# rohitgandikota/sliders

Measured on AMD Instinct MI355X. Metric: UNet denoise steps/sec (SDXL rank-4 text slider), higher is better.
Workload: dtype bf16; 1 GPU; sdxl text slider rank=4 alpha=1 noxattn+c3lier, 1024x1024, batch 1 (CFG pair), DDIM-50 partial denoise k~U{1..49} + 4 predictions + backward + AdamW; bench_step=one training iteration, prompt_pairs=8, parallelism=dp1

## Files before the change

### sliders_amd/csrc/lora.hip

```cpp
#include "addressing.h"
#include "../../include/sliders_hip.h"

namespace {

struct AddrArgs {
    const __bf16* a0; const __bf16* a1;
    int lda0, lda1, ca0, ca1;
    int mode, hs, ws, src_xform, stride, ho, wo;
};

template <int RMAX, int LPR>
__global__ __launch_bounds__(256) void skinny_kernel(AddrArgs A, const __bf16* __restrict__ w,
                                                     const __bf16* __restrict__ bias, void* out,
                                                     int M, int R, int K, int ldo, int out_kind, int kmajor) {
    const int tid = threadIdx.x;
    const int sub = tid & (LPR - 1);
    const int m = blockIdx.x * (256 / LPR) + tid / LPR;
    const bool active = m < M;
    const int mm = active ? m : M - 1;
    float acc[RMAX];
#pragma unroll
    for (int r = 0; r < RMAX; ++r) acc[r] = 0.f;
    const int cin = A.ca0 + A.ca1;

    auto fma_chunk = [&](const bf16x8 x, int k) {
        float xf[8];
#pragma unroll
        for (int e = 0; e < 8; ++e) xf[e] = (float)x[e];
        if (kmajor) {
            if (RMAX == 4) {
#pragma unroll
                for (int h = 0; h < 4; ++h) {
                    const bf16x8 wv = *(const bf16x8*)(w + (long)k * 4 + h * 8);
#pragma unroll
                    for (int r = 0; r < 4; ++r) {
                        acc[r] += xf[2 * h] * (float)wv[r];
                        acc[r] += xf[2 * h + 1] * (float)wv[4 + r];
                    }
                }
            }
            return;
        }
        bf16x8 wv[RMAX];
#pragma unroll
        for (int r = 0; r < RMAX; ++r) wv[r] = *(const bf16x8*)(w + (long)(r < R ? r : 0) * K + k);
#pragma unroll
        for (int r = 0; r < RMAX; ++r) {
            if (r < R) {
#pragma unroll
                for (int e = 0; e < 8; ++e) acc[r] += xf[e] * (float)wv[r][e];
            }
        }
    };

    if (A.mode == 0) {
        auto src_of = [&](int k) {
            const int kc = k < K ? k : 0;
            return kc < A.ca0 ? A.a0 + (long)mm * A.lda0 + kc : A.a1 + (long)mm * A.lda1 + (kc - A.ca0);
        };
        bf16x8 cur = *(const bf16x8*)src_of(sub * 8);
        for (int k = sub * 8; k < K; k += LPR * 8) {
            const bf16x8 nxt = *(const bf16x8*)src_of(k + LPR * 8);
            fma_chunk(cur, k);
            cur = nxt;
        }
    } else {
        const int hw = A.ho * A.wo;
        const int b = mm / hw;
        const int rem = mm - b * hw;
        const int oy = rem / A.wo, ox = rem - oy * A.wo;
        const int sh = A.src_xform ? 1 : 0;
        const int HL = A.hs << sh, WL = A.ws << sh;
        for (int tap = 0; tap < 9; ++tap) {
            const int ky = tap / 3, kx = tap - ky * 3;
            const int iy = oy * A.stride + ky - 1, ix = ox * A.stride + kx - 1;
            bool ok = (iy >= 0) & (iy < HL) & (ix >= 0) & (ix < WL);
            if (A.src_xform == 2) ok = ok & (((iy | ix) & 1) == 0);
            if (!ok) continue;
            const long pix = ((long)b * A.hs + (iy >> sh)) * A.ws + (ix >> sh);
            auto src_of = [&](int c) {
                const int cc = c < cin ? c : 0;
                return cc < A.ca0 ? A.a0 + pix * A.lda0 + cc : A.a1 + pix * A.lda1 + (cc - A.ca0);
            };
            bf16x8 cur = *(const bf16x8*)src_of(sub * 8);
            for (int c = sub * 8; c < cin; c += LPR * 8) {
                const bf16x8 nxt = *(const bf16x8*)src_of(c + LPR * 8);
                fma_chunk(cur, tap * cin + c);
                cur = nxt;
            }
        }
    }
#pragma unroll
    for (int r = 0; r < RMAX; ++r) {
#pragma unroll
        for (int o = LPR / 2; o > 0; o >>= 1) acc[r] += __shfl_xor(acc[r], o, 64);
    }
    if (active && sub == 0) {
        if (out_kind == 0) {
            float* o = (float*)out + (long)m * ldo;
#pragma unroll
            for (int r = 0; r < RMAX; ++r)
                if (r < R) o[r] = acc[r] + (bias ? (float)bias[r] : 0.f);
        } else {
            const int hw = A.ho * A.wo;
            const int b = m / hw;
            const int rem = m - b * hw;
            __bf16* o = (__bf16*)out;
#pragma unroll
            for (int r = 0; r < RMAX; ++r)
                if (r < R) o[((long)b * R + r) * hw + rem] = (__bf16)(acc[r] + (bias ? (float)bias[r] : 0.f));
        }
    }
}

__global__ __launch_bounds__(256) void gemv_kernel(const slh_gemv_desc d) {
    const int lane = threadIdx.x & 63;
    const int n = blockIdx.x * 4 + (threadIdx.x >> 6);
    if (n >= d.N) return;
    const __bf16* x = (const __bf16*)d.x;
    const __bf16* w = (const __bf16*)d.w + (long)n * d.K;
    float acc[8];
#pragma unroll
    for (int b = 0; b < 8; ++b) acc[b] = 0.f;
    for (int k = lane * 8; k < d.K; k += 512) {
        const bf16x8 wv = *(const bf16x8*)(w + k);
        bf16x8 xv[8];
#pragma unroll
        for (int b = 0; b < 8; ++b) xv[b] = *(const bf16x8*)(x + (long)(b < d.nb ? b : d.nb - 1) * d.ldx + k);
        float wf[8];
#pragma unroll
        for (int e = 0; e < 8; ++e) wf[e] = (float)wv[e];
#pragma unroll
        for (int b = 0; b < 8; ++b) {
            if (b < d.nb) {
#pragma unroll
                for (int e = 0; e < 8; ++e) {
                    float xe = (float)xv[b][e];
                    if (d.in_act == 1) xe = round_bf16(silu_f(xe));
                    acc[b] += xe * wf[e];
                }
            }
        }
    }
#pragma unroll
    for (int b = 0; b < 8; ++b) acc[b] = wave_sum(acc[b]);
    if (lane == 0) {
        const float bias = d.bias ? (float)((const __bf16*)d.bias)[n] : 0.f;
        float up[4] = {0.f, 0.f, 0.f, 0.f};
        float ls = 0.f;
        int tcol = 0;
        if (d.lora_t) {
            ls = *d.lora_scale;
            tcol = d.lora_tcol ? d.lora_tcol[n] : 0;
            const bf16x4 u = *(const bf16x4*)((const __bf16*)d.lora_up + (long)n * 4);
#pragma unroll
            for (int r = 0; r < 4; ++r) up[r] = (float)u[r];
        }
        for (int b = 0; b < d.nb; ++b) {
            float v = acc[b] + bias;
            if (d.lora_t) {
                const float* t = d.lora_t + (long)b * d.ld_t + tcol;
                v += ls * (t[0] * up[0] + t[1] * up[1] + t[2] * up[2] + t[3] * up[3]);
            }
            if (d.addend) v = round_bf16(v) + (float)((const __bf16*)d.addend)[(long)b * d.ld_add + n];
            if (d.out_f32) ((float*)d.y)[(long)b * d.ldy + n] = v;
            else ((__bf16*)d.y)[(long)b * d.ldy + n] = (__bf16)v;
        }
    }
}

struct WgradArgs {
    AddrArgs A;
    const float* v; float* out; const float* scale;
    int M, R, ldv, ldo, rows_per_block, rmajor, vgroup_cols;
    float* ws; unsigned* ticket;
};

template <int R>
__device__ __forceinline__ void wgrad_body(const WgradArgs& p, const int bx, const int by, const int bz, const long slab_id = 0,
                                           const int slab_step = 0, const long ticket_id = 0, const int splits = 1) {
    __shared__ float red[4][32][8 * R + 1];
    __shared__ int last_flag;
    const int cx = threadIdx.x & 31, ry = threadIdx.x >> 5;
    const int C = p.A.ca0 + p.A.ca1;
    const int c = (bx * 32 + cx) * 8;
    const bool cvalid = c < C;
    const int tap = bz;
    const int m_begin = by * p.rows_per_block;
    const int m_end = min(p.M, m_begin + p.rows_per_block);
    float acc[8][R];
#pragma unroll
    for (int e = 0; e < 8; ++e)
#pragma unroll
        for (int r = 0; r < R; ++r) acc[e][r] = 0.f;
    const int voff = p.vgroup_cols > 0 ? 4 * (c / p.vgroup_cols) : 0;
    const int ky = tap / 3, kx = tap - ky * 3;
    const SrcSel zs = src_select(p.A, c);
    if (cvalid) {
        for (int m = m_begin + ry; m < m_end; m += 8) {
            long pix = m;
            if (p.A.mode != 0) {
                const RowPixel px = pixel_of_row(m, p.A.ho, p.A.wo);
                const ConvTap t = conv_tap(p.A, px.b, px.oy, px.ox, ky, kx);
                if (!t.ok) continue;
                pix = t.pix;
            }
            const bf16x8 z = *(const bf16x8*)(zs.base + pix * zs.ld + zs.cc);
            float vv[R];
#pragma unroll
            for (int r = 0; r < R; ++r) vv[r] = p.v[(long)m * p.ldv + voff + r];
#pragma unroll
            for (int e = 0; e < 8; ++e) {
                const float ze = (float)z[e];
#pragma unroll
                for (int r = 0; r < R; ++r) acc[e][r] += ze * vv[r];
            }
        }
    }
#pragma unroll
    for (int e = 0; e < 8; ++e)
#pragma unroll
        for (int r = 0; r < R; ++r) {
            acc[e][r] += __shfl_xor(acc[e][r], 32, 64);
            if ((threadIdx.x & 32) == 0) red[threadIdx.x >> 6][cx][e * R + r] = acc[e][r];
        }
    __syncthreads();
    const float s = *p.scale;
    if (p.ws != nullptr) {
        constexpr int PER = 32 * 8 * R;
        const __amdgpu_buffer_rsrc_t slabs = __builtin_amdgcn_make_buffer_rsrc(p.ws + slab_id * PER - (long)by * slab_step * PER, 0,
                                                                              (int)((long)splits * slab_step * PER * 4), 0x00020000);
#pragma unroll
        for (int q = 0; q < PER / 1024; ++q) {
            const int idx = (q * 256 + threadIdx.x) * 4;
            f32x4 t4;
#pragma unroll
            for (int u = 0; u < 4; ++u) {
                const int ccx = (idx + u) / (8 * R), er = (idx + u) - ccx * (8 * R);
                float t = 0.f;
#pragma unroll
                for (int y = 0; y < 4; ++y) t += red[y][ccx][er];
                t4[u] = t;
            }
            __builtin_amdgcn_raw_buffer_store_b128(__builtin_bit_cast(u32x4, t4), slabs, (by * slab_step * PER + idx) * 4, 0, 16 );
        }
        if (!last_arriver(p.ticket + ticket_id, (unsigned)splits, &last_flag)) return;
#pragma unroll
        for (int q = 0; q < PER / 1024; ++q) {
            const int idx = (q * 256 + threadIdx.x) * 4;
            f32x4 tot = {0.f, 0.f, 0.f, 0.f};
            for (int k0 = 0; k0 < splits; k0 += 8) {
                f32x4 v[8];
#pragma unroll
                for (int u = 0; u < 8; ++u)
                    v[u] = k0 + u < splits ? __builtin_bit_cast(f32x4, __builtin_amdgcn_raw_buffer_load_b128(
                                                 slabs, ((k0 + u) * slab_step * PER + idx) * 4, 0, 16 ))
                                           : f32x4{0.f, 0.f, 0.f, 0.f};
#pragma unroll
                for (int u = 0; u < 8; ++u) tot += v[u];
            }
#pragma unroll
            for (int u = 0; u < 4; ++u) {
                const int ccx = (idx + u) / (8 * R), er = (idx + u) - ccx * (8 * R);
                const int e = er / R, r = er - e * R;
                const int cc = (bx * 32 + ccx) * 8 + e;
                if (cc >= C) continue;
                const long col = (p.A.mode == 0 ? 0 : (long)tap * C) + cc;
                float* o = p.rmajor ? p.out + (long)r * p.ldo + col : p.out + col * p.ldo + r;
                *o += s * tot[u];
            }
        }
        return;
    }
    for (int idx = threadIdx.x; idx < 32 * 8 * R; idx += 256) {
        const int ccx = idx / (8 * R);
        const int er = idx - ccx * (8 * R);
        const int e = er / R, r = er - e * R;
        const int cc = (bx * 32 + ccx) * 8 + e;
        if (cc >= C) continue;
        float t = 0.f;
#pragma unroll
        for (int y = 0; y < 4; ++y) t += red[y][ccx][er];
        const long col = (p.A.mode == 0 ? 0 : (long)tap * C) + cc;
        float* o = p.rmajor ? p.out + (long)r * p.ldo + col : p.out + col * p.ldo + r;
        atomicAdd(o, s * t);
    }
}

template <int R>
__global__ __launch_bounds__(256) void wgrad_kernel(const WgradArgs p) {
    wgrad_body<R>(p, blockIdx.x, blockIdx.y, blockIdx.z, ((long)blockIdx.z * gridDim.y + blockIdx.y) * gridDim.x + blockIdx.x,
                  (int)gridDim.x, (long)blockIdx.z * gridDim.x + blockIdx.x, (int)gridDim.y);
}

struct WgradGeom { int gx, splits, taps, rows_per_block; };
__host__ __device__ inline WgradGeom wgrad_geom(int C, int M, int mode, int kind) {
    WgradGeom g;
    g.gx = (C / 8 + 31) / 32;
    g.taps = mode == 1 ? 9 : 1;
    const int blocks_xz = g.gx * g.taps;
    const int target = kind == 0 ? 768 : 256;
    int splits = kind == 2 ? (M + 511) / 512 : (target + blocks_xz - 1) / blocks_xz;
    const int max_splits = (M + 63) / 64, min_splits = kind == 2 ? 1 : (M + 1023) / 1024;
    if (splits > max_splits) splits = max_splits;
    if (splits < min_splits) splits = min_splits;
    if (splits < 1) splits = 1;
    g.splits = splits;
    g.rows_per_block = ((M + splits - 1) / splits + 7) / 8 * 8;
    return g;
}

__host__ __device__ inline void fill_addr(AddrArgs& A, const void* a0, const void* a1, int lda0, int lda1, int ca0, int ca1, int mode,
                                         int hs, int ws, int src_xform, int stride, int ho, int wo) {
    A.a0 = (const __bf16*)a0; A.a1 = (const __bf16*)a1;
    A.lda0 = lda0; A.lda1 = lda1; A.ca0 = ca0; A.ca1 = ca1; A.mode = mode;
    A.hs = hs; A.ws = ws; A.src_xform = src_xform; A.stride = stride; A.ho = ho; A.wo = wo;
}

__host__ __device__ inline void wgrad_args(WgradArgs& p, const slh_wgrad_desc& d) {
    fill_addr(p.A, d.z0, d.z1, d.ldz0, d.ldz1, d.c0, d.c1, d.mode, d.hs, d.ws, d.src_xform, d.stride, d.ho, d.wo);
    p.v = d.v; p.out = d.out; p.scale = d.scale;
    p.M = d.M; p.R = d.R; p.ldv = d.ldv; p.ldo = d.ldo;
    p.rmajor = d.out_rmajor;
    p.vgroup_cols = d.vgroup_cols;
    p.ws = d.slabs; p.ticket = (unsigned*)d.tickets;
    p.rows_per_block = wgrad_geom(d.c0 + d.c1, d.M, d.mode, d.slabs ? 1 : 0).rows_per_block;
}

template <int R>
__global__ __launch_bounds__(256) void wgrad_batch_kernel(const slh_wgrad_desc* table, const int* prefix, int n, float* ws, unsigned* ticket) {
    const int bid = blockIdx.x;
    const int pi = __builtin_amdgcn_readfirstlane(batch_find(prefix, n, bid));
    const slh_wgrad_desc d = table[pi];
    WgradArgs p;
    wgrad_args(p, d);
    p.ws = ws; p.ticket = ticket;
    const WgradGeom g = wgrad_geom(d.c0 + d.c1, d.M, d.mode, ws ? 2 : 0);
    p.rows_per_block = g.rows_per_block;
    const int local = bid - prefix[pi];
    const int bx = local % g.gx, rest = local / g.gx;
    const int by = rest % g.splits, bz = rest / g.splits;
    wgrad_body<R>(p, bx, by, bz, bid, g.gx, (long)prefix[pi] + (long)bz * g.splits * g.gx + bx, g.splits);
}

}

struct skinny_form { int rmax, lpr, grid; };
static skinny_form skinny_choose(int M, int R) {
    skinny_form f;
    f.rmax = R <= 4 ? 4 : R <= 12 ? 12 : 16;
    f.lpr = M <= 16384 ? 64 : 16;
    const int rows = 256 / f.lpr;
    f.grid = (M + rows - 1) / rows;
    return f;
}

extern "C" int slh_skinny(const slh_skinny_desc* d, slh_stream_t stream) {
    SLH_CHECK(d && d->a0 && d->w && d->out, "slh_skinny: null pointer");
    SLH_CHECK(d->M > 0 && d->R > 0 && d->R <= 16 && d->K > 0, "slh_skinny: bad shape");
    SLH_CHECK(d->ca0 % 8 == 0 && d->ca1 % 8 == 0 && d->lda0 % 8 == 0 && d->lda1 % 8 == 0 && d->K % 8 == 0,
              "slh_skinny: 16-byte alignment");
    SLH_CHECK((d->a1 != nullptr) == (d->ca1 > 0), "slh_skinny: a1/ca1 mismatch");
    const int cin = d->ca0 + d->ca1;
    if (d->mode == 0) SLH_CHECK(cin == d->K, "slh_skinny: dense K mismatch");
    else {
        SLH_CHECK(d->mode == 1 && d->K == 9 * cin, "slh_skinny: conv K mismatch");
        SLH_CHECK(d->M == d->batch * d->ho * d->wo, "slh_skinny: conv M mismatch");
        SLH_CHECK(d->stride == 1 || d->stride == 2, "slh_skinny: stride");
    }
    if (d->out_kind == 1) SLH_CHECK(d->mode == 1, "slh_skinny: NCHW output needs conv geometry");
    if (d->w_kmajor) SLH_CHECK(d->R == 4 && d->mode == 0 && !d->bias, "slh_skinny: w_kmajor needs dense R=4");
    AddrArgs A;
    fill_addr(A, d->a0, d->a1, d->lda0, d->lda1, d->ca0, d->ca1, d->mode, d->hs, d->ws, d->src_xform, d->stride,
              d->ho, d->wo);
    hipStream_t s = (hipStream_t)stream;
    const skinny_form f = skinny_choose(d->M, d->R);
#define SLH_SKINNY_LAUNCH(RM, LPR)                                                                                 \
    do {                                                                                                           \
        if (slh_name_mode()) slh_name_record("skinny<%d,%d>", RM, LPR);                                            \
        else                                                                                                       \
            hipLaunchKernelGGL((skinny_kernel<RM, LPR>), dim3(f.grid), dim3(256), 0, s, A, (const __bf16*)d->w,    \
                               (const __bf16*)d->bias, d->out, d->M, d->R, d->K, d->ldo, d->out_kind, d->w_kmajor); \
    } while (0)
#define SLH_SKINNY_ROWS(RM)                                                                                        \
    do {                                                                                                           \
        if (f.lpr == 64) SLH_SKINNY_LAUNCH(RM, 64);                                                                \
        else SLH_SKINNY_LAUNCH(RM, 16);                                                                            \
    } while (0)
    if (f.rmax == 4) SLH_SKINNY_ROWS(4);
    else if (f.rmax == 12) SLH_SKINNY_ROWS(12);
    else SLH_SKINNY_ROWS(16);
#undef SLH_SKINNY_ROWS
#undef SLH_SKINNY_LAUNCH
    SLH_LAUNCH_CHECK("slh_skinny");
    return 0;
}

extern "C" int slh_skinny_kernel_name(const slh_skinny_desc* d, char* buf, int cap) {
    SLH_CHECK(buf && cap >= 32, "slh_skinny_kernel_name: buffer");
    slh_name_sink_set(buf, cap);
    const int rc = slh_skinny(d, nullptr);
    slh_name_sink_set(nullptr, 0);
    if (rc == 0 && !buf[0]) { slh_set_error("slh_skinny_kernel_name: internal: no launch site recorded a name"); return -3; }
    return rc;
}

extern "C" int slh_gemv(const slh_gemv_desc* d, slh_stream_t stream) {
    SLH_CHECK(d && d->x && d->w && d->y, "slh_gemv: null pointer");
    SLH_CHECK(d->nb >= 1 && d->nb <= 8 && d->N > 0 && d->K > 0 && d->K % 8 == 0 && d->ldx % 8 == 0,
              "slh_gemv: bad shape nb=%d N=%d K=%d", d->nb, d->N, d->K);
    if (d->lora_t) SLH_CHECK(d->lora_up && d->lora_scale, "slh_gemv: lora pointers");
    hipLaunchKernelGGL(gemv_kernel, dim3((d->N + 3) / 4), dim3(256), 0, (hipStream_t)stream, *d);
    SLH_LAUNCH_CHECK("slh_gemv");
    return 0;
}

static int wgrad_check(const slh_wgrad_desc* d, bool ptrs = true) {
    SLH_CHECK(d, "slh_lora_wgrad: null descriptor");
    if (ptrs) SLH_CHECK(d->z0 && d->v && d->out && d->scale, "slh_lora_wgrad: null pointer");
    SLH_CHECK(d->R == 4 || d->R == 12, "slh_lora_wgrad: R must be 4 or 12");
    SLH_CHECK(d->c0 % 8 == 0 && d->c1 % 8 == 0 && d->ldz0 % 8 == 0 && d->ldz1 % 8 == 0, "slh_lora_wgrad: alignment");
    if (ptrs) SLH_CHECK((d->z1 != nullptr) == (d->c1 > 0), "slh_lora_wgrad: z1/c1 mismatch");
    SLH_CHECK(d->M > 0 && d->c0 + d->c1 > 0, "slh_lora_wgrad: empty problem");
    if (d->mode == 1) SLH_CHECK(d->M == d->batch * d->ho * d->wo, "slh_lora_wgrad: conv M mismatch");
    if (d->vgroup_cols > 0)
        SLH_CHECK(d->vgroup_cols % 8 == 0 && (d->c0 + d->c1) % d->vgroup_cols == 0 && d->R == 4,
                  "slh_lora_wgrad: vgroup_cols %d needs a multiple of 8 that divides C = %d, and R = 4 (R = %d)", d->vgroup_cols,
                  d->c0 + d->c1, d->R);
    SLH_CHECK(d->vgroup_cols >= 0, "slh_lora_wgrad: negative vgroup_cols");
    return 0;
}

extern "C" int slh_lora_wgrad(const slh_wgrad_desc* d, slh_stream_t stream) {
    if (wgrad_check(d)) return -1;
    WgradArgs p;
    wgrad_args(p, *d);
    SLH_CHECK((d->slabs != nullptr) == (d->tickets != nullptr), "slh_lora_wgrad: slabs and tickets come together");
    const WgradGeom g = wgrad_geom(d->c0 + d->c1, d->M, d->mode, d->slabs ? 1 : 0);
    dim3 grid(g.gx, g.splits, g.taps);
    hipStream_t s = (hipStream_t)stream;
    if (d->R == 4) hipLaunchKernelGGL(wgrad_kernel<4>, grid, dim3(256), 0, s, p);
    else hipLaunchKernelGGL(wgrad_kernel<12>, grid, dim3(256), 0, s, p);
    SLH_LAUNCH_CHECK("slh_lora_wgrad");
    return 0;
}

extern "C" int slh_lora_wgrad_blocks(const slh_wgrad_desc* d) {
    if (wgrad_check(d, false)) return -1;
    const WgradGeom g = wgrad_geom(d->c0 + d->c1, d->M, d->mode, d->slabs ? 2 : 0);
    return g.gx * g.splits * g.taps;
}

extern "C" int slh_lora_wgrad_single_blocks(const slh_wgrad_desc* d) {
    if (wgrad_check(d, false)) return -1;
    const WgradGeom g = wgrad_geom(d->c0 + d->c1, d->M, d->mode, 1);
    return g.gx * g.splits * g.taps;
}

extern "C" int slh_lora_wgrad_geometry(const slh_wgrad_desc* d, int kind, int32_t* out4) {
    if (wgrad_check(d, false)) return -1;
    SLH_CHECK(kind >= 0 && kind <= 2 && out4, "slh_lora_wgrad_geometry: kind must be 0, 1 or 2");
    const WgradGeom g = wgrad_geom(d->c0 + d->c1, d->M, d->mode, kind);
    out4[0] = g.gx; out4[1] = g.splits; out4[2] = g.taps; out4[3] = g.rows_per_block;
    return 0;
}

extern "C" int slh_lora_wgrad_batch(const slh_batch_desc* d, slh_stream_t stream) {
    SLH_CHECK(d && d->table && d->prefix && d->n > 0 && d->total > 0, "slh_lora_wgrad_batch: empty batch / null pointer");
    SLH_CHECK(d->arg == 4 || d->arg == 12, "slh_lora_wgrad_batch: arg must be the common R (4 or 12)");
    SLH_CHECK((d->slabs != nullptr) == (d->tickets != nullptr), "slh_lora_wgrad_batch: slabs and tickets come together");
    hipStream_t s = (hipStream_t)stream;
    if (d->arg == 4)
        hipLaunchKernelGGL(wgrad_batch_kernel<4>, dim3(d->total), dim3(256), 0, s, (const slh_wgrad_desc*)d->table, d->prefix, d->n,
                           (float*)d->slabs, (unsigned*)d->tickets);
    else
        hipLaunchKernelGGL(wgrad_batch_kernel<12>, dim3(d->total), dim3(256), 0, s, (const slh_wgrad_desc*)d->table, d->prefix, d->n,
                           (float*)d->slabs, (unsigned*)d->tickets);
    SLH_LAUNCH_CHECK("slh_lora_wgrad_batch");
    return 0;
}

namespace {
__global__ __launch_bounds__(256) void lora_conv_dgrad_kernel(const slh_lora_cdgrad_desc d) {
    const int nchunk = d.cin / 8;
    const long gid = (long)blockIdx.x * blockDim.x + threadIdx.x;
    const long total = (long)d.batch * d.hl * d.wl * nchunk;
    if (gid >= total) return;
    const int chunk = (int)(gid % nchunk);
    const long pix = gid / nchunk;
    const int hw = d.hl * d.wl;
    const int b = (int)(pix / hw);
    const int rem = (int)(pix - (long)b * hw);
    const int iy = rem / d.wl, ix = rem - iy * d.wl;
    const int c = chunk * 8;
    const __bf16* A = (const __bf16*)d.a_down;
    const int K = 9 * d.cin;
    float acc[8];
#pragma unroll
    for (int e = 0; e < 8; ++e) acc[e] = 0.f;
    for (int tap = 0; tap < 9; ++tap) {
        const int ky = tap / 3, kx = tap - ky * 3;
        const int ty = iy + 1 - ky, tx = ix + 1 - kx;
        if (ty < 0 || tx < 0) continue;
        if (d.stride == 2 && ((ty | tx) & 1)) continue;
        const int oy = ty / d.stride, ox = tx / d.stride;
        if (oy >= d.ho || ox >= d.wo) continue;
        const f32x4 u = *(const f32x4*)(d.u + ((long)b * d.ho * d.wo + (long)oy * d.wo + ox) * d.ldu);
#pragma unroll
        for (int r = 0; r < 4; ++r) {
            const bf16x8 a = *(const bf16x8*)(A + (long)r * K + tap * d.cin + c);
#pragma unroll
            for (int e = 0; e < 8; ++e) acc[e] += u[r] * (float)a[e];
        }
    }
    const float s = *d.scale;
    __bf16* g = (__bf16*)d.gx + pix * d.ldgx + c;
    bf16x8 o;
    if (d.accumulate) o = *(const bf16x8*)g;
#pragma unroll
    for (int e = 0; e < 8; ++e) o[e] = (__bf16)(s * acc[e] + (d.accumulate ? (float)o[e] : 0.f));
    *(bf16x8*)g = o;
}

__global__ __launch_bounds__(256) void temb_lora_bwd_kernel(const slh_temb_lora_bwd_desc d) {
    __shared__ float red[4][4];
    __shared__ float U[4];
    const int tid = threadIdx.x;
    const float s = *d.scale;
    float t[4], part[4] = {0.f, 0.f, 0.f, 0.f};
#pragma unroll
    for (int r = 0; r < 4; ++r) t[r] = d.t[r];
    for (int c = tid; c < d.C; c += 256) {
        const float g = d.g[c];
        const bf16x4 u = *(const bf16x4*)((const __bf16*)d.up + (long)c * 4);
#pragma unroll
        for (int r = 0; r < 4; ++r) {
            part[r] += g * (float)u[r];
            d.d_up[(long)c * 4 + r] += s * g * t[r];
        }
    }
#pragma unroll
    for (int r = 0; r < 4; ++r) part[r] = wave_sum(part[r]);
    if ((tid & 63) == 0) {
#pragma unroll
        for (int r = 0; r < 4; ++r) red[tid >> 6][r] = part[r];
    }
    __syncthreads();
    if (tid < 4) U[tid] = red[0][tid] + red[1][tid] + red[2][tid] + red[3][tid];
    __syncthreads();
    for (int k = tid; k < d.ted; k += 256) {
        const float x = round_bf16(silu_f((float)((const __bf16*)d.emb)[k]));
#pragma unroll
        for (int r = 0; r < 4; ++r) d.d_down[(long)r * d.ted + k] += s * U[r] * x;
    }
}
__global__ __launch_bounds__(256) void lora_ln_fold_kernel(const slh_lora_lnfold_item* items) {
    const slh_lora_lnfold_item it = items[blockIdx.y];
    const int r = blockIdx.x;
    if (r >= it.rows) return;
    __shared__ float red[2][4];
    const int tid = threadIdx.x;
    const __bf16* a = (const __bf16*)it.a + (long)r * it.K;
    __bf16* o = (__bf16*)it.a_out + (long)r * it.K;
    float s = 0.f, c = 0.f;
    for (int k = tid * 8; k < it.K; k += 256 * 8) {
        const bf16x8 av = *(const bf16x8*)(a + k);
        const bf16x8 gv = *(const bf16x8*)((const __bf16*)it.gamma + k);
        const bf16x8 bv = *(const bf16x8*)((const __bf16*)it.beta + k);
        bf16x8 ov;
#pragma unroll
        for (int e = 0; e < 8; ++e) {
            ov[e] = (__bf16)((float)av[e] * (float)gv[e]);
            s += (float)ov[e];
            c += (float)av[e] * (float)bv[e];
        }
        *(bf16x8*)(o + k) = ov;
    }
    s = wave_sum(s);
    c = wave_sum(c);
    if ((tid & 63) == 0) { red[0][tid >> 6] = s; red[1][tid >> 6] = c; }
    __syncthreads();
    if (tid == 0) {
        it.s_out[r] = (red[0][0] + red[0][1]) + (red[0][2] + red[0][3]);
        it.c_out[r] = (red[1][0] + red[1][1]) + (red[1][2] + red[1][3]);
    }
}
}

extern "C" int slh_lora_ln_fold(const slh_lora_lnfold_desc* d, slh_stream_t stream) {
    SLH_CHECK(d && d->items && d->n > 0, "slh_lora_ln_fold: null pointer / empty");
    hipLaunchKernelGGL(lora_ln_fold_kernel, dim3(16, d->n), dim3(256), 0, (hipStream_t)stream, d->items);
    SLH_LAUNCH_CHECK("slh_lora_ln_fold");
    return 0;
}

extern "C" int slh_lora_conv_dgrad(const slh_lora_cdgrad_desc* d, slh_stream_t stream) {
    SLH_CHECK(d && d->u && d->a_down && d->scale && d->gx, "slh_lora_conv_dgrad: null pointer");
    SLH_CHECK(d->cin % 8 == 0 && d->ldgx % 8 == 0 && d->ldu % 4 == 0 && (d->stride == 1 || d->stride == 2),
              "slh_lora_conv_dgrad: bad shape");
    const long total = (long)d->batch * d->hl * d->wl * (d->cin / 8);
    hipLaunchKernelGGL(lora_conv_dgrad_kernel, dim3((unsigned)((total + 255) / 256)), dim3(256), 0, (hipStream_t)stream, *d);
    SLH_LAUNCH_CHECK("slh_lora_conv_dgrad");
    return 0;
}

extern "C" int slh_temb_lora_bwd(const slh_temb_lora_bwd_desc* d, slh_stream_t stream) {
    SLH_CHECK(d && d->g && d->t && d->up && d->emb && d->d_up && d->d_down && d->scale, "slh_temb_lora_bwd: null pointer");
    hipLaunchKernelGGL(temb_lora_bwd_kernel, dim3(1), dim3(256), 0, (hipStream_t)stream, *d);
    SLH_LAUNCH_CHECK("slh_temb_lora_bwd");
    return 0;
}
```

### sliders_amd/trainer.py

```python
from __future__ import annotations

import ctypes as C
from dataclasses import dataclass
from itertools import count
from typing import Optional

import os

import torch

from . import lib
from . import schedulers
from .ddim import DDIMSchedule
from .lora_store import LoraStore
from .parallel import allreduce_sum_, world_info
from .passes import Pass, default_time_ids
from .unet import UNetEngine

TENSOR_OP_OPTIMIZERS = ("prodigy", "dadaptadam", "dadaptlion")


@dataclass
class PairEmbeds:
    ctx_target: torch.Tensor
    ctx_positive: torch.Tensor
    ctx_neutral: torch.Tensor
    ctx_uncond: torch.Tensor
    pooled_target: Optional[torch.Tensor] = None
    pooled_positive: Optional[torch.Tensor] = None
    pooled_neutral: Optional[torch.Tensor] = None
    pooled_uncond: Optional[torch.Tensor] = None
    guidance_scale: float = 1.0
    action: str = "enhance"


def _stream() -> int:
    return torch.cuda.current_stream().cuda_stream


class _ShapeState:

    def __init__(self, cfg, bs: int, H: int, W: int, dev):
        shape = (bs, cfg.out_channels, H, W)
        z = lambda: torch.zeros(shape, dtype=torch.bfloat16, device=dev)
        self.denoised, self.e_pos, self.e_neu, self.e_unc, self.e_tgt = z(), z(), z(), z(), z()
        self.chw = cfg.out_channels * H * W
        self.time_ids = None
        if cfg.is_xl:
            self.time_ids = default_time_ids(H, W, 2 * bs).to(dev)


class _StepPrograms:

    def __init__(self, tr: "SliderTrainer", p_on, key):
        self.key, self.tr, self.drv = key, tr, Pass(tr.eng, p_on)
        B = 2 * tr.bs
        n = len(tr.t50)
        self.t_table = torch.tensor([[float(t)] * B for t in tr.t50], dtype=torch.float32, device=tr.eng.device).reshape(n, B)
        self.progs = [None] * n
        self.captured = False

    def program(self, i: int) -> lib.Program:
        pr = self.progs[i]
        if pr is not None:
            return pr
        tr, p = self.tr, self.drv.p
        base = self.drv.program(i == 0)
        t_io = p.io["t"].ptr
        pr = lib.Program()
        patched = 0
        for (op, d), nm in zip(base.ops, base.op_names):
            if op == lib.OP_TEMBED and d.vals == t_io:
                d = lib.TembedDesc.from_buffer_copy(bytes(d))
                d.vals = self.t_table.data_ptr() + i * self.t_table.shape[1] * 4
                patched += 1
            pr.add(op, d, nm)
        if patched != 1:
            raise RuntimeError(f"step program: {patched} timestep projections read io['t'] (expected one)")
        smp = p.io["sample"]
        half = tr.bs * tr.chw * 2
        pr.add(lib.OP_CFG_DDIM, tr._cfg_desc(p, smp.ptr, tr.denoise_guidance, tr.sched.step_fields(tr.t50[i], tr.nsteps),
                                             out2=smp.ptr + half, x=smp.ptr), "cfg_ddim_step")
        self.progs[i] = pr
        return pr

    def capture_all(self):
        if self.captured:
            return
        self.captured = True
        for i in range(max(1, self.tr.nsteps - 1)):
            if not self.program(i).capture():
                break


class SliderTrainer:
    def __init__(self, engine: UNetEngine, store: LoraStore, H: int, W: int, batch_size: int = 1,
                 lr: float = 2e-4, betas=(0.9, 0.999), eps: float = 1e-8, weight_decay: float = 0.01,
                 max_denoising_steps: int = 50, denoise_guidance: float = 3.0, process_group=None,
                 dedup_frozen: bool = True, prediction_type: str = "epsilon", optimizer: str = "adamw",
                 noise_scheduler: str = "ddim", scheduler_seed: int = 0, optimizer_kwargs: Optional[dict] = None):
        self.eng, self.store = engine, store
        self.lr, self.betas, self.eps, self.wd = lr, betas, eps, weight_decay
        if optimizer not in ("adamw", "adam", "lion") + TENSOR_OP_OPTIMIZERS:
            raise NotImplementedError(f"optimizer '{optimizer}': fused flat kernels exist for adam / adamw (slh_adamw) and lion "
                                      f"(slh_lion); prodigy / dadaptadam / dadaptlion run as sliders_amd.optim classes on the flat "
                                      f"parameter buffer")
        if getattr(store, "master", None) is not None and optimizer not in ("adamw", "adam"):
            raise NotImplementedError(f"optimizer '{optimizer}' with fp32 adapter state (train.precision: float32): only the fused "
                                      f"adam / adamw kernel keeps an fp32 master; use bfloat16 for lion / prodigy / dadapt*")
        self.optimizer = optimizer
        self.optimizer_kwargs = dict(optimizer_kwargs or {})
        self._tensor_opt = None
        self.nsteps = max_denoising_steps
        self.denoise_guidance = denoise_guidance
        if noise_scheduler.lower().replace(" ", "_") == "ddim":
            self.sched = DDIMSchedule(prediction_type=prediction_type)
        else:
            self.sched = schedulers.create(noise_scheduler, prediction_type)
            self.sched_generator = torch.Generator(device=engine.device)
            self.sched_generator.manual_seed(int(scheduler_seed))
        self.pg = process_group
        self.rank, self.world = world_info(process_group)
        self.time_allreduce = False
        self._ar_events = []
        self.grad_scale = 1.0
        engine.attach_lora(store) if engine.lora is not store else None
        self.loss = torch.zeros(1, dtype=torch.float32, device=engine.device)
        if self.sched.fused:
            self.t50 = self.sched.make_timesteps(max_denoising_steps)
            self.t1000 = self.sched.make_timesteps(1000)
        self.unet_passes = 0
        self.dedup_frozen = dedup_frozen
        self.overlap_frozen = os.environ.get("SLIDERS_OVERLAP_FROZEN", "1") == "1"
        self._side = torch.cuda.Stream(device=engine.device) if self.overlap_frozen else None
        self.step_graphs = os.environ.get("SLIDERS_STEP_GRAPHS", "1") == "1"
        self.frozen_gate = int(os.environ.get("SLIDERS_FROZEN_GATE", "1"))
        self._captured = set()
        self.phase_events = None
        self.phase_steps = False
        self._states = {}
        self._use(batch_size, H, W)

    def _use(self, bs: int, H: int, W: int):
        key = (bs, H, W)
        st = self._states.get(key)
        if st is None:
            st = self._states[key] = _ShapeState(self.eng.cfg, bs, H, W, self.eng.device)
        self.H, self.W, self.bs = H, W, bs
        self.denoised, self.e_pos, self.e_neu, self.e_unc, self.e_tgt = st.denoised, st.e_pos, st.e_neu, st.e_unc, st.e_tgt
        self.chw, self.time_ids = st.chw, st.time_ids

    def _begin(self, noise, lr, time_ids):
        self._use(noise.shape[0], noise.shape[2], noise.shape[3])
        if time_ids is not None:
            self.time_ids = time_ids.to(device=self.eng.device, dtype=torch.float32).reshape(2 * self.bs, 6)
        if lr is not None:
            self.lr = float(lr)

    def _model_input(self, lat, t):
        return lat if self.sched.fused else self.sched.scale_model_input(lat, t)

    def _denoise_unfused(self, drv: Pass, noise, k: int):
        sch, s = self.sched, _stream()
        eps = self.e_tgt
        step = count()

        def predict(model_input, t):
            drv.load_latents(model_input)
            drv.run(t, next(step) == 0, s)
            self.unet_passes += 1
            self._cfg(drv.p, eps.data_ptr(), self.denoise_guidance)
            return eps

        lat = schedulers.denoise(sch, predict, noise.to(device=self.eng.device, dtype=torch.bfloat16), k, self.nsteps,
                                 generator=self.sched_generator, device=self.eng.device)
        self.denoised.copy_(lat)
        sch.set_timesteps(1000, device=self.eng.device)
        return sch.timesteps[int(k * 1000 / self.nsteps)]

    def _cfg_desc(self, p, out, guidance, coeff=None, out2=None, x=None, eps_text=None):
        d = lib.CfgDdimDesc(eps=p.io["eps"].ptr, x=x or 0, out=out, out2=out2 or 0, eps_text=eps_text or 0,
                            nb=self.bs, chw=self.chw, guidance=guidance, do_step=0)
        if coeff is not None:
            for kf, vf in coeff.items():
                setattr(d, kf, vf)
        return d

    def _cfg(self, p, out, guidance, coeff=None, out2=None, x=None, eps_text=None):
        lib.call(lib.OP_CFG_DDIM, self._cfg_desc(p, out, guidance, coeff, out2, x, eps_text), _stream())

    def _step_programs(self, p_on) -> "_StepPrograms":
        key = (id(self), self.bs, self.chw, self.nsteps, float(self.denoise_guidance))
        sp = getattr(p_on, "_step_progs", None)
        if sp is None or sp.key != key:
            sp = p_on._step_progs = _StepPrograms(self, p_on, key)
        return sp

    def _predict(self, p, lat, ctx, pooled, t, out):
        drv = Pass(self.eng, p)
        drv.load_latents(self._model_input(lat, t))
        drv.load_cond(ctx, pooled, self.time_ids)
        drv.run(t, True, _stream())
        self.unet_passes += 1
        self._cfg(p, out.data_ptr(), 1.0)

    def _frozen_dedup(self, pair: PairEmbeds, t_cur: int):
        eng, bs = self.eng, self.bs
        p3 = eng.plan(3 * bs, self.H, self.W, "off")
        drv = Pass(eng, p3)
        drv.load_latents(self._model_input(self.denoised, t_cur))
        ctx = p3.io["ctx"].tensor
        ctx[:bs].copy_(pair.ctx_uncond[:bs]); ctx[bs:2 * bs].copy_(pair.ctx_positive[bs:]); ctx[2 * bs:].copy_(pair.ctx_neutral[bs:])
        if eng.cfg.is_xl:
            p3.io["time_ids"].tensor.copy_(self.time_ids[:1].expand(3 * bs, 6))
            ai = p3.io["add_in"].tensor
            pd = eng.cfg.pooled_dim
            ai[:bs, :pd].copy_(pair.pooled_uncond[:bs]); ai[bs:2 * bs, :pd].copy_(pair.pooled_positive[bs:])
            ai[2 * bs:, :pd].copy_(pair.pooled_neutral[bs:])
        drv.run(t_cur, True, _stream())
        self.unet_passes += 3
        e = p3.io["eps"].ptr
        blk = bs * self.chw * 2
        self._cfg(p3, self.e_pos.data_ptr(), 1.0, eps_text=e + blk)
        self._cfg(p3, self.e_neu.data_ptr(), 1.0, eps_text=e + 2 * blk)
        self._cfg(p3, self.e_unc.data_ptr(), 1.0, eps_text=e)

    def iteration(self, pair: PairEmbeds, k: int, noise: torch.Tensor, lr: Optional[float] = None,
                  time_ids: Optional[torch.Tensor] = None, zero_grads: bool = True, step: bool = True) -> torch.Tensor:
        self._mark("start")
        self._begin(noise, lr, time_ids)
        eng, st, bs = self.eng, self.store, self.bs
        B = 2 * bs
        s = _stream()
        gate = None
        eng.set_lora(True, 1.0)
        p_on = eng.plan(B, self.H, self.W, "on")
        drv = Pass(eng, p_on)
        drv.load_cond(pair.ctx_target, pair.pooled_target, self.time_ids)
        if self.sched.fused:
            drv.load_latents(noise)
            smp = p_on.io["sample"]
            half = bs * self.chw * 2
            sp = self._step_programs(p_on) if self.step_graphs else None
            gate_at = k - self.frozen_gate if (self.overlap_frozen and self.frozen_gate > 0) else -1
            for i in range(k):
                self.unet_passes += 1
                if i == gate_at:
                    gate = torch.cuda.Event()
                    gate.record(torch.cuda.current_stream())
                if sp is not None:
                    sp.program(i).run(s)
                    if self.phase_events is not None and self.phase_steps:
                        self._mark(f"step{i}")
                    continue
                t = self.t50[i]
                drv.run(t, i == 0, s)
                self._cfg(p_on, smp.ptr, self.denoise_guidance, self.sched.step_fields(t, self.nsteps),
                          out2=smp.ptr + half, x=smp.ptr)
            if sp is not None:
                sp.capture_all()
            self._mark("denoise")
            self.denoised.copy_(smp.tensor[:bs])
            t_cur = self.t1000[int(k * 1000 / self.nsteps)]
        else:
            t_cur = self._denoise_unfused(drv, noise, k)
        def frozen():
            if self.dedup_frozen:
                self._frozen_dedup(pair, t_cur)
            else:
                p_off = eng.plan(B, self.H, self.W, "off")
                self._predict(p_off, self.denoised, pair.ctx_positive, pair.pooled_positive, t_cur, self.e_pos)
                self._predict(p_off, self.denoised, pair.ctx_neutral, pair.pooled_neutral, t_cur, self.e_neu)
                self._predict(p_off, self.denoised, pair.ctx_uncond, pair.pooled_uncond, t_cur, self.e_unc)

        eng.set_lora(False)
        frozen_done = None
        if self.overlap_frozen:
            eng.plan(3 * bs if self.dedup_frozen else B, self.H, self.W, "off")
            eng.plan(B, self.H, self.W, "train")
            main = torch.cuda.current_stream()
            if gate is not None:
                gate.synchronize()
            self._side.wait_stream(main)
            with torch.cuda.stream(self._side):
                frozen()
                frozen_done = torch.cuda.Event()
                frozen_done.record(self._side)
        else:
            frozen()
        eng.set_lora(True, 1.0)
        p_tr = eng.plan(B, self.H, self.W, "train")
        self._predict(p_tr, self.denoised, pair.ctx_target, pair.pooled_target, t_cur, self.e_tgt)
        if frozen_done is not None:
            torch.cuda.current_stream().wait_event(frozen_done)
        self._mark("predictions")
        self.loss.zero_()
        bw = p_tr.backward
        n = bs * self.chw
        d = lib.LossDesc(target=self.e_tgt.data_ptr(), positive=self.e_pos.data_ptr(), neutral=self.e_neu.data_ptr(),
                         uncond=self.e_unc.data_ptr(), loss=self.loss.data_ptr(), dtarget=0,
                         dtarget_pix=bw.deps_pix.ptr, n=n, guidance=float(pair.guidance_scale),
                         erase=1 if pair.action == "erase" else 0, hw=self.H * self.W, nch=eng.cfg.out_channels)
        lib.call(lib.OP_LOSS, d, s)
        if zero_grads:
            st.grads.zero_()
        bw.prog.run(s)
        self._mark("backward")
        if step:
            self.reduce_and_step()
            self._mark("optimizer")
        if self.step_graphs:
            key = (B, self.H, self.W, self.dedup_frozen)
            if key not in self._captured:
                self._captured.add(key)
                off = eng.plan(3 * bs if self.dedup_frozen else B, self.H, self.W, "off")
                for prog in (off.prog, p_tr.prog, bw.prog):
                    if prog._runs >= 1:
                        prog.capture()
        return self.loss

    def _mark(self, name: str):
        if self.phase_events is not None:
            e = torch.cuda.Event(enable_timing=True)
            e.record(torch.cuda.current_stream())
            self.phase_events.append((name, e))

    def reduce_and_step(self, n_accumulated: int = 1):
        st = self.store
        cur = torch.cuda.current_stream()
        timed = self.time_allreduce and (self.pg is not None or self.world > 1)
        if timed:
            e0, e1 = torch.cuda.Event(enable_timing=True), torch.cuda.Event(enable_timing=True)
            e0.record(cur)
        self.grad_scale = allreduce_sum_(st.grads, self.pg) / float(n_accumulated)
        if timed:
            e1.record(cur)
            self._ar_events.append((e0, e1))
        self.optimizer_step()

    def allreduce_ms(self):
        out = [a.elapsed_time(b) for a, b in self._ar_events]
        self._ar_events = []
        return out

    def optimizer_step(self):
        st = self.store
        st.opt_step += 1
        if self.optimizer in TENSOR_OP_OPTIMIZERS:
            if self._tensor_opt is None:
                from . import optim
                cls = {"prodigy": optim.Prodigy, "dadaptadam": optim.DAdaptAdam, "dadaptlion": optim.DAdaptLion}[self.optimizer]
                kw = {k: v for k, v in self.optimizer_kwargs.items()}
                if self.eps and self.optimizer != "dadaptlion":
                    kw.setdefault("eps", self.eps)
                self._tensor_opt = cls([st.params], lr=self.lr, betas=self.betas, weight_decay=self.wd, **kw)
            self._tensor_opt.param_groups[0]["lr"] = self.lr
            st.params.grad = (st.grads * self.grad_scale).to(st.params.dtype)
            self._tensor_opt.step()
            st.params.grad = None
            return
        if self.optimizer == "lion":
            d = lib.LionDesc(param=st.params.data_ptr(), exp_avg=st.exp_avg.data_ptr(), grad=st.grads.data_ptr(), n=st.numel,
                             lr=self.lr, beta1=self.betas[0], beta2=self.betas[1], weight_decay=self.wd,
                             grad_scale=self.grad_scale)
            lib.call(lib.OP_LION, d, _stream())
            return
        f32 = st.master is not None
        d = lib.AdamwDesc(param=(st.master if f32 else st.params).data_ptr(), exp_avg=st.exp_avg.data_ptr(),
                          exp_avg_sq=st.exp_avg_sq.data_ptr(), grad=st.grads.data_ptr(), n=st.numel, lr=self.lr, beta1=self.betas[0],
                          beta2=self.betas[1], eps=self.eps, weight_decay=self.wd, step=st.opt_step, grad_scale=self.grad_scale,
                          param_lo=st.params.data_ptr() if f32 else 0, f32_state=1 if f32 else 0)
        lib.call(lib.OP_ADAMW, d, _stream())
```

Before: 47.00 steps/s.

## Hoist timestep conditioning branch out of denoise loop into one batched prelude

Before the denoise loop, the time/add embedding branch (time_proj, embedding linears, LoRA temb down, time_emb_proj_all) is computed once for all k steps with nb=k*B rows. The per-step programs then skip those ops and point each resnet's row-bias at the precomputed slice for that step. This removes many small per-step GEMV launches in exchange for one larger batched pass. A new multi-row GEMV kernel supports nb>8 by keeping weights in registers across row groups, and it limits K to 3072.

After: 47.08 steps/s (median of 6 runs). Within noise of the previous version (+0.2%).

```diff
diff --git a/sliders_amd/csrc/lora.hip b/sliders_amd/csrc/lora.hip
--- a/sliders_amd/csrc/lora.hip
+++ b/sliders_amd/csrc/lora.hip
@@ -158,6 +158,89 @@
         }
         for (int b = 0; b < d.nb; ++b) {
             float v = acc[b] + bias;
+            if (d.lora_t) {
+                const float* t = d.lora_t + (long)b * d.ld_t + tcol;
+                v += ls * (t[0] * up[0] + t[1] * up[1] + t[2] * up[2] + t[3] * up[3]);
+            }
+            if (d.addend) v = round_bf16(v) + (float)((const __bf16*)d.addend)[(long)b * d.ld_add + n];
+            if (d.out_f32) ((float*)d.y)[(long)b * d.ldy + n] = v;
+            else ((__bf16*)d.y)[(long)b * d.ldy + n] = (__bf16)v;
+        }
+    }
+}
+
+constexpr int GEMV_NW = 4;
+template <int KF>
+__global__ __launch_bounds__(256) void gemv_rows_kernel(const slh_gemv_desc d) {
+    const int lane = threadIdx.x & 63;
+    const int n0 = (blockIdx.x * 4 + (threadIdx.x >> 6)) * GEMV_NW;
+    if (n0 >= d.N) return;
+    const __bf16* x = (const __bf16*)d.x;
+    bf16x8 wv[GEMV_NW][KF];
+#pragma unroll
+    for (int j = 0; j < GEMV_NW; ++j) {
+        const int nj = n0 + j < d.N ? n0 + j : d.N - 1;
+#pragma unroll
+        for (int f = 0; f < KF; ++f) {
+            const int k = lane * 8 + 512 * f;
+            wv[j][f] = *(const bf16x8*)((const __bf16*)d.w + (long)nj * d.K + (k < d.K ? k : 0));
+        }
+    }
+    const int eb = lane & 7, ej = lane >> 3;
+    const int en = n0 + ej;
+    const bool elane = ej < GEMV_NW && en < d.N;
+    const int n = elane ? en : n0;
+    const float bias = d.bias ? (float)((const __bf16*)d.bias)[n] : 0.f;
+    float up[4] = {0.f, 0.f, 0.f, 0.f};
+    float ls = 0.f;
+    int tcol = 0;
+    if (d.lora_t) {
+        ls = *d.lora_scale;
+        tcol = d.lora_tcol ? d.lora_tcol[n] : 0;
+        const bf16x4 u = *(const bf16x4*)((const __bf16*)d.lora_up + (long)n * 4);
+#pragma unroll
+        for (int r = 0; r < 4; ++r) up[r] = (float)u[r];
+    }
+    for (int r0 = 0; r0 < d.nb; r0 += 8) {
+        float acc[GEMV_NW][8];
+#pragma unroll
+        for (int j = 0; j < GEMV_NW; ++j)
+#pragma unroll
+            for (int b = 0; b < 8; ++b) acc[j][b] = 0.f;
+#pragma unroll
+        for (int f = 0; f < KF; ++f) {
+            const int k = lane * 8 + 512 * f;
+            const bool kok = k < d.K;
+            bf16x8 xv[8];
+#pragma unroll
+            for (int b = 0; b < 8; ++b)
+                xv[b] = *(const bf16x8*)(x + (long)(r0 + b < d.nb ? r0 + b : d.nb - 1) * d.ldx + (kok ? k : 0));
+            if (kok) {
+#pragma unroll
+                for (int b = 0; b < 8; ++b) {
+                    if (r0 + b < d.nb) {
+#pragma unroll
+                        for (int e = 0; e < 8; ++e) {
+                            float xe = (float)xv[b][e];
+                            if (d.in_act == 1) xe = round_bf16(silu_f(xe));
+#pragma unroll
+                            for (int j = 0; j < GEMV_NW; ++j) acc[j][b] += xe * (float)wv[j][f][e];
+                        }
+                    }
+                }
+            }
+        }
+        float mine = 0.f;
+#pragma unroll
+        for (int j = 0; j < GEMV_NW; ++j)
+#pragma unroll
+            for (int b = 0; b < 8; ++b) {
+                const float s = wave_sum(acc[j][b]);
+                if (lane == j * 8 + b) mine = s;
+            }
+        const int b = r0 + eb;
+        if (elane && b < d.nb) {
+            float v = mine + bias;
             if (d.lora_t) {
                 const float* t = d.lora_t + (long)b * d.ld_t + tcol;
                 v += ls * (t[0] * up[0] + t[1] * up[1] + t[2] * up[2] + t[3] * up[3]);
@@ -407,9 +490,19 @@
 
 extern "C" int slh_gemv(const slh_gemv_desc* d, slh_stream_t stream) {
     SLH_CHECK(d && d->x && d->w && d->y, "slh_gemv: null pointer");
-    SLH_CHECK(d->nb >= 1 && d->nb <= 8 && d->N > 0 && d->K > 0 && d->K % 8 == 0 && d->ldx % 8 == 0,
+    SLH_CHECK(d->nb >= 1 && d->N > 0 && d->K > 0 && d->K % 8 == 0 && d->ldx % 8 == 0,
               "slh_gemv: bad shape nb=%d N=%d K=%d", d->nb, d->N, d->K);
     if (d->lora_t) SLH_CHECK(d->lora_up && d->lora_scale, "slh_gemv: lora pointers");
+    if (d->nb > 8) {
+        SLH_CHECK(d->K <= 512 * 6, "slh_gemv: nb=%d > 8 rows need K <= 3072 (K=%d)", d->nb, d->K);
+        const dim3 grid((d->N + 4 * GEMV_NW - 1) / (4 * GEMV_NW));
+        const int kf = (d->K + 511) / 512;
+        if (kf <= 1) hipLaunchKernelGGL(gemv_rows_kernel<1>, grid, dim3(256), 0, (hipStream_t)stream, *d);
+        else if (kf <= 3) hipLaunchKernelGGL(gemv_rows_kernel<3>, grid, dim3(256), 0, (hipStream_t)stream, *d);
+        else hipLaunchKernelGGL(gemv_rows_kernel<6>, grid, dim3(256), 0, (hipStream_t)stream, *d);
+        SLH_LAUNCH_CHECK("slh_gemv");
+        return 0;
+    }
     hipLaunchKernelGGL(gemv_kernel, dim3((d->N + 3) / 4), dim3(256), 0, (hipStream_t)stream, *d);
     SLH_LAUNCH_CHECK("slh_gemv");
     return 0;
diff --git a/sliders_amd/trainer.py b/sliders_amd/trainer.py
--- a/sliders_amd/trainer.py
+++ b/sliders_amd/trainer.py
@@ -50,6 +50,75 @@
             self.time_ids = default_time_ids(H, W, 2 * bs).to(dev)
 
 
+class _LoopConditioning:
+
+    OPS = ("time_proj", "time_embedding.linear_1", "time_embedding.linear_2", "add_time_proj", "add_embedding.linear_1",
+           "add_embedding.linear_2", "temb.lora_down", "time_emb_proj_all")
+
+    def __init__(self, p, t_table: torch.Tensor):
+        self.p, self.t_table = p, t_table
+        self.n, self.B = t_table.shape
+        rows, dev = self.n * self.B, t_table.device
+        self.base = [(op, d, nm) for (op, d), nm in zip(p.prog.ops, p.prog.op_names) if nm in self.OPS]
+        if [nm for _, _, nm in self.base][-1:] != ["time_emb_proj_all"] or self.base[0][2] != "time_proj":
+            raise RuntimeError(f"loop conditioning: unexpected branch {[nm for _, _, nm in self.base]}")
+        self.bufs = {}
+        self.tid = None
+        for op, d, nm in self.base:
+            if op == lib.OP_TEMBED:
+                self._rows_of(d.out, d.ldo, torch.bfloat16, rows, dev)
+                if d.vals != p.io["t"].ptr:
+                    if d.vals != p.io["time_ids"].ptr:
+                        raise RuntimeError(f"loop conditioning: {nm} reads neither io['t'] nor io['time_ids']")
+                    self.tid = torch.zeros((rows, d.n_vals), dtype=torch.float32, device=dev)
+            else:
+                self._rows_of(d.y, d.ldy, torch.float32 if d.out_f32 else torch.bfloat16, rows, dev)
+        self.table = self.bufs[p.temb_all.ptr].view(self.n, self.B, p.temb_all.shape[1])
+        self._preludes = {}
+
+    def _rows_of(self, ptr, ld, dtype, rows, dev):
+        if ptr not in self.bufs:
+            self.bufs[ptr] = torch.zeros((rows, ld), dtype=dtype, device=dev)
+
+    def _moved(self, ptr: int, nm: str) -> int:
+        if not ptr:
+            return 0
+        if ptr not in self.bufs:
+            raise RuntimeError(f"loop conditioning: {nm} reads a buffer that the branch does not write")
+        return self.bufs[ptr].data_ptr()
+
+    def prelude(self, k: int) -> lib.Program:
+        pr = self._preludes.get(k)
+        if pr is None:
+            pr = self._preludes[k] = lib.Program()
+            for op, d, nm in self.base:
+                d = type(d).from_buffer_copy(bytes(d))
+                d.nb = k * self.B
+                if op == lib.OP_TEMBED:
+                    d.vals = self.t_table.data_ptr() if self.tid is None or d.vals == self.p.io["t"].ptr else self.tid.data_ptr()
+                    d.out = self._moved(d.out, nm)
+                else:
+                    d.x, d.addend, d.lora_t, d.y = (self._moved(v, nm) for v in (d.x, d.addend, d.lora_t, d.y))
+                pr.add(op, d, nm)
+        return pr
+
+    def begin(self, k: int, stream: int):
+        io = self.p.io
+        if self.tid is not None:
+            pd = self.p.cfg.pooled_dim
+            ai = io["add_in"]
+            self.tid.view(self.n, self.B, -1)[:k].copy_(io["time_ids"].tensor)
+            self.bufs[ai.ptr].view(self.n, self.B, -1)[:k, :, :pd].copy_(ai.tensor[:, :pd])
+        self.prelude(k).run(stream)
+
+    def rowbias_in_step(self, ptr: int, i: int) -> Optional[int]:
+        ta = self.p.temb_all
+        off = ptr - ta.ptr
+        if not 0 <= off < self.B * ta.shape[1] * 2:
+            return None
+        return self.table.data_ptr() + i * self.B * ta.shape[1] * 2 + off
+
+
 class _StepPrograms:
 
     def __init__(self, tr: "SliderTrainer", p_on, key):
@@ -58,7 +127,9 @@
         n = len(tr.t50)
         self.t_table = torch.tensor([[float(t)] * B for t in tr.t50], dtype=torch.float32, device=tr.eng.device).reshape(n, B)
         self.progs = [None] * n
+        self.loop_progs = [None] * n
         self.captured = False
+        self.cond = _LoopConditioning(p_on, self.t_table) if tr.loop_temb else None
 
     def program(self, i: int) -> lib.Program:
         pr = self.progs[i]
@@ -84,12 +155,38 @@
         self.progs[i] = pr
         return pr
 
+    def loop_program(self, i: int) -> lib.Program:
+        pr = self.loop_progs[i]
+        if pr is not None:
+            return pr
+        full, cond = self.program(i), self.cond
+        pr = lib.Program()
+        biases = 0
+        for (op, d), nm in zip(full.ops, full.op_names):
+            if nm in cond.OPS:
+                continue
+            if op == lib.OP_GEMM and d.rowbias:
+                rb = cond.rowbias_in_step(d.rowbias, i)
+                if rb is not None:
+                    d = lib.GemmDesc.from_buffer_copy(bytes(d))
+                    d.rowbias = rb
+                    biases += 1
+            pr.add(op, d, nm)
+        n_res = len(self.drv.p.w.resnet_paths)
+        if biases != n_res:
+            raise RuntimeError(f"step program: {biases} products read their row bias from temb.proj_all, the net has {n_res} resnets")
+        self.loop_progs[i] = pr
+        return pr
+
+    def step(self, i: int) -> lib.Program:
+        return self.program(i) if self.cond is None else self.loop_program(i)
+
     def capture_all(self):
         if self.captured:
             return
         self.captured = True
         for i in range(max(1, self.tr.nsteps - 1)):
-            if not self.program(i).capture():
+            if not self.program(i).capture() or (self.cond is not None and not self.loop_program(i).capture()):
                 break
 
 
@@ -134,6 +231,7 @@
         self.overlap_frozen = os.environ.get("SLIDERS_OVERLAP_FROZEN", "1") == "1"
         self._side = torch.cuda.Stream(device=engine.device) if self.overlap_frozen else None
         self.step_graphs = os.environ.get("SLIDERS_STEP_GRAPHS", "1") == "1"
+        self.loop_temb = os.environ.get("SLIDERS_LOOP_TEMB", "1") == "1"
         self.frozen_gate = int(os.environ.get("SLIDERS_FROZEN_GATE", "1"))
         self._captured = set()
         self.phase_events = None
@@ -190,7 +288,7 @@
         lib.call(lib.OP_CFG_DDIM, self._cfg_desc(p, out, guidance, coeff, out2, x, eps_text), _stream())
 
     def _step_programs(self, p_on) -> "_StepPrograms":
-        key = (id(self), self.bs, self.chw, self.nsteps, float(self.denoise_guidance))
+        key = (id(self), self.bs, self.chw, self.nsteps, float(self.denoise_guidance), self.loop_temb)
         sp = getattr(p_on, "_step_progs", None)
         if sp is None or sp.key != key:
             sp = p_on._step_progs = _StepPrograms(self, p_on, key)
@@ -242,6 +340,8 @@
             smp = p_on.io["sample"]
             half = bs * self.chw * 2
             sp = self._step_programs(p_on) if self.step_graphs else None
+            if sp is not None and sp.cond is not None:
+                sp.cond.begin(k, s)
             gate_at = k - self.frozen_gate if (self.overlap_frozen and self.frozen_gate > 0) else -1
             for i in range(k):
                 self.unet_passes += 1
@@ -249,7 +349,7 @@
                     gate = torch.cuda.Event()
                     gate.record(torch.cuda.current_stream())
                 if sp is not None:
-                    sp.program(i).run(s)
+                    sp.step(i).run(s)
                     if self.phase_events is not None and self.phase_steps:
                         self._mark(f"step{i}")
                     continue
```
